# OpenDrift/opendrift

Measured on AMD Instinct MI355X. Metric: particle-steps/sec (RK4, 3D interp), higher is better.
Workload: dtype f64; 1 GPU; C3: OceanDrift 3D, synthetic ROMS-shaped z-level grid 1024x1024x12 (u,v,w,K), RK4 + vertical_mixing(60 s) + vertical_advection; particles_per_gpu=10000000, particles_total=10000000, stage_math=fast, spin_up_steps=200, block_every=0, inputs=resident in HBM, parallelism=particle-sharded x1, field block broadcast once per time level

## Files before the change

include/odrift.h:

```cpp
#ifndef ODRIFT_H
#define ODRIFT_H
#include <stdint.h>

#ifdef __cplusplus
extern "C" {
#endif

typedef struct odr_ctx odr_ctx;
typedef struct odr_particles odr_particles;

typedef enum {
  ODR_OK = 0,
  ODR_ERR_INVALID = -1,
  ODR_ERR_HIP = -2,
  ODR_ERR_CAPACITY = -3,
  ODR_ERR_STATE = -4
} odr_status;

enum {
  ODR_VAR_X_SEA_WATER_VELOCITY = 0,
  ODR_VAR_Y_SEA_WATER_VELOCITY = 1,
  ODR_VAR_X_WIND = 2,
  ODR_VAR_Y_WIND = 3,
  ODR_VAR_UPWARD_SEA_WATER_VELOCITY = 4,
// ... 252 lines not shown
                         const double *depth_noise, uint64_t step);
int odr_radio_terminal_velocity(odr_ctx *ctx, odr_particles *p, int diameter_slot, int density_slot);
int odr_radio_resuspend(odr_ctx *ctx, odr_particles *p, odr_radio *radio, int specie_slot, int diameter_slot, int rng_mode,
                        const double *diameter_noise, const double *depth_noise, uint64_t step);
int odr_particles_count_status(odr_ctx *ctx, odr_particles *p, int32_t status_code, int64_t *n);
int odr_particles_remap_status(odr_ctx *ctx, odr_particles *p, int32_t from_code, int32_t to_code);
int odr_deactivate(odr_ctx *ctx, odr_particles *p, const uint8_t *mask_host, int32_t status_code);
int odr_deactivate_outside(odr_ctx *ctx, odr_particles *p, double west, double east, double south, double north,
                           int32_t status_code);
int odr_compact(odr_ctx *ctx, odr_particles *p, int64_t *n_active);
int odr_scan_status(odr_ctx *ctx, odr_particles *p, int64_t *n_kept, uint64_t *status_flags);
int odr_scan_status_begin(odr_ctx *ctx, odr_particles *p);
int odr_scan_status_end(odr_ctx *ctx, odr_particles *p, int64_t *n_kept, uint64_t *status_flags);
int odr_ctx_guard_next_vmix(odr_ctx *ctx, int on);
int odr_compact_apply(odr_ctx *ctx, odr_particles *p, int64_t *n_active);
int odr_sort_particles(odr_ctx *ctx, odr_particles *p, int32_t source_id);
int odr_sort_particles_ex(odr_ctx *ctx, odr_particles *p, int32_t source_id, int keep_environment);
int odr_particles_tile_stats(odr_ctx *ctx, odr_particles *p, uint64_t *out4);
int odr_particles_step_layout_stats(odr_ctx *ctx, odr_particles *p, uint64_t *out2);
int odr_particles_step_onlevel_stats(odr_ctx *ctx, odr_particles *p, uint64_t *out1);
int odr_particles_vmix_layout_stats(odr_ctx *ctx, odr_particles *p, uint64_t *out3);
int odr_particles_vmix_kplane_stats(odr_ctx *ctx, odr_particles *p, uint64_t *out2);
int odr_particles_vmix_window_stats(odr_ctx *ctx, odr_particles *p, uint64_t *out3);
int odr_reduce_scalars(odr_ctx *ctx, odr_particles *p, double wind_drift_depth, double *out16);
int odr_ctx_set_step_reduce(odr_ctx *ctx, int on, double wind_drift_depth, int relative_wind);
int odr_reduce_local(odr_ctx *ctx, odr_particles *p, double wind_drift_depth, int relative_wind, double *out16);
int odr_reduce_install(odr_ctx *ctx, odr_particles *p, const double *in16);
int odr_reduce_unpin(odr_ctx *ctx);

int odr_ctx_set_position_class(odr_ctx *ctx, int f32);
int odr_source_set_coordinate_dtype(odr_ctx *ctx, int32_t source_id, int x_is_float32, int y_is_float32);

#define ODR_COMM_ID_BYTES 256
int odr_device_count(int32_t *n);
int odr_comm_unique_id(uint8_t *id );
int odr_comm_init(odr_ctx *ctx, const uint8_t *id, int32_t rank, int32_t nranks);
int odr_comm_info(int32_t *rank, int32_t *nranks, uint64_t *id_hash, int32_t *rccl_version, uint64_t *collectives);
int odr_comm_destroy(void);
int odr_allreduce_scalars(odr_ctx *ctx, double *values, int32_t n, int32_t op);
int odr_comm_allgather_begin(odr_ctx *ctx, const double *row, int32_t n, int32_t from_scan);
int odr_comm_allgather_end(odr_ctx *ctx, double *rows );
int odr_comm_broadcast_bytes(odr_ctx *ctx, void *buf, int64_t nbytes, int32_t root);
int odr_comm_barrier(odr_ctx *ctx);
int odr_block_broadcast(odr_ctx *ctx, int32_t source_id, int32_t slot, double t_epoch, int nvars, const int32_t *var_ids,
                        const void *const *data, const int32_t *var_nz, int ny, int nx, const double *xy8, int32_t root);

// ... 107 lines not shown
```

opendrift_amd/_abi.py:

```python
import ctypes as C
import os

HERE = os.path.dirname(os.path.abspath(__file__))
LIB_PATH = os.environ.get('ODR_LIB') or os.path.join(HERE, 'libodrift_hip.so')

NVAR = 26
VARIABLES = {
    'x_sea_water_velocity': 0, 'y_sea_water_velocity': 1, 'x_wind': 2, 'y_wind': 3,
    'upward_sea_water_velocity': 4, 'ocean_vertical_diffusivity': 5,
    'sea_surface_wave_stokes_drift_x_velocity': 6, 'sea_surface_wave_stokes_drift_y_velocity': 7,
    'land_binary_mask': 8, 'sea_floor_depth_below_sea_level': 9, 'sea_surface_height': 10,
    'horizontal_diffusivity': 11, 'sea_surface_wave_significant_height': 12,
    'sea_surface_wave_period_at_variance_spectral_density_maximum': 13,
    'ocean_mixed_layer_thickness': 14,
    'sea_water_temperature': 15, 'sea_water_salinity': 16,
    'sea_ice_area_fraction': 17, 'sea_ice_x_velocity': 18, 'sea_ice_y_velocity': 19,
    'sea_surface_swell_wave_to_direction': 20,
    'sea_surface_swell_wave_peak_period_from_variance_spectral_density': 21,
    'sea_surface_swell_wave_significant_height': 22, 'sea_surface_wind_wave_to_direction': 23,
    'sea_surface_wind_wave_mean_period': 24, 'sea_surface_wind_wave_significant_height': 25,
}
VARIABLE_NAMES = {v: k for k, v in VARIABLES.items()}
PROJ_LATLONG, PROJ_STERE_EQUIT_SPHERE, PROJ_STERE_POLAR = 0, 1, 2
PROJ_MERC, PROJ_LCC = 4, 5
# ... 158 lines not shown
    'odr_comm_unique_id': [_P(C.c_uint8)],
    'odr_comm_init': [_vp, _P(C.c_uint8), C.c_int32, C.c_int32],
    'odr_comm_info': [_P(C.c_int32), _P(C.c_int32), _P(C.c_uint64), _P(C.c_int32), _P(C.c_uint64)],
    'odr_comm_destroy': [],
    'odr_allreduce_scalars': [_vp, _dp, C.c_int32, C.c_int32],
    'odr_comm_allgather_begin': [_vp, _dp, C.c_int32, C.c_int32],
    'odr_comm_allgather_end': [_vp, _dp],
    'odr_comm_broadcast_bytes': [_vp, _vp, C.c_int64, C.c_int32],
    'odr_comm_barrier': [_vp],
    'odr_block_broadcast': [_vp, C.c_int32, C.c_int32, C.c_double, C.c_int, _ip, _P(_vp), _ip, C.c_int, C.c_int, _dp, C.c_int32],
    'odr_scan_status': [_vp, _vp, _i64p, _P(C.c_uint64)],
    'odr_scan_status_begin': [_vp, _vp],
    'odr_scan_status_end': [_vp, _vp, _i64p, _P(C.c_uint64)],
    'odr_ctx_guard_next_vmix': [_vp, C.c_int],
    'odr_compact_apply': [_vp, _vp, _i64p],
    'odr_sort_particles': [_vp, _vp, C.c_int32],
    'odr_sort_particles_ex': [_vp, _vp, C.c_int32, C.c_int],
    'odr_particles_tile_stats': [_vp, _vp, _P(C.c_uint64)],
    'odr_particles_step_layout_stats': [_vp, _vp, _P(C.c_uint64)],
    'odr_particles_step_onlevel_stats': [_vp, _vp, _P(C.c_uint64)],
    'odr_particles_vmix_layout_stats': [_vp, _vp, _P(C.c_uint64)],
    'odr_particles_vmix_kplane_stats': [_vp, _vp, _P(C.c_uint64)],
    'odr_particles_vmix_window_stats': [_vp, _vp, _P(C.c_uint64)],
    'odr_reduce_scalars': [_vp, _vp, C.c_double, _dp],
    'odr_ctx_set_step_reduce': [_vp, C.c_int, C.c_double, C.c_int],
    'odr_reduce_local': [_vp, _vp, C.c_double, C.c_int, _dp],
    'odr_reduce_install': [_vp, _vp, _dp],
    'odr_reduce_unpin': [_vp],
    'odr_timer_begin': [_vp],
    'odr_timer_end': [_vp, _fp],
    'odr_sgrid_create': [_vp, C.c_int32, C.c_int32, C.c_int32, _dp, _dp, C.c_double, _dp, _dp, C.c_int32, _P(_vp)],
    'odr_sgrid_destroy': [_vp, _vp],
    'odr_sgrid_download_zrho': [_vp, _vp, _dp],
    'odr_sgrid_zslice': [_vp, _vp, _vp, C.c_int, C.c_int, C.c_int32, _dp, C.c_int32, _P(_vp), _dp],
    'odr_history_create': [_vp, C.c_int64, C.c_int32, C.c_int32, _ip, _P(_vp)],
    'odr_history_destroy': [_vp, _vp],
    'odr_history_set_id_base': [_vp, _vp, C.c_int64],
    'odr_history_record': [_vp, _vp, _vp, C.c_int32, C.c_int, C.c_int],
    'odr_history_flush': [_vp, _vp, C.c_int32, C.c_int32],
    'odr_history_wait': [_vp, _vp],
    'odr_history_host_ptr': [_vp, _vp, C.c_int32, _P(_fp), _P(C.c_int32)],
    'odr_history_reset': [_vp, _vp],
    'odr_history_minmax': [_vp, _vp, C.c_int32, _dp, _dp],
    'odr_density_map': [_vp, C.c_int64, C.c_int32] + [_vp] * 5 + [C.c_int32, C.c_int32, _dp, C.c_int32, _dp, _dp, _dp, _dp],
    'odr_density_last_kernel_ms': [_vp, _fp],
    'odr_density_map_proj': [_vp, C.c_int64, C.c_int32] + [_vp] * 5 + [C.c_int32, _P(ProjDesc), C.c_int32, _dp, C.c_int32, _dp, C.c_int64, _dp, _dp, _dp],
# ... 81 lines not shown
```

opendrift_amd/build.py:

```python
import os
import subprocess
from concurrent.futures import ThreadPoolExecutor

HERE = os.path.dirname(os.path.abspath(__file__))
CSRC = os.path.join(HERE, 'csrc')
UNITS = sorted(f for f in os.listdir(CSRC) if f.endswith('.hip'))
HEADERS = sorted(os.path.join(CSRC, f) for f in os.listdir(CSRC) if f.endswith('.h')) + \
    [os.path.join(os.path.dirname(HERE), 'include', 'odrift.h')]
LIB = os.path.join(HERE, 'libodrift_hip.so')
OBJDIR = os.path.join(HERE, 'build')
HIPCC = os.environ.get('HIPCC', '/opt/rocm/bin/hipcc')
FLAGS = ['--offload-arch=gfx950', '-O3', '-std=c++17', '-ffp-contract=off', '-fPIC',
         '-I' + os.path.join(os.path.dirname(HERE), 'include')]


def _stale(target, deps):
    return not os.path.exists(target) or any(os.path.getmtime(target) < os.path.getmtime(d) for d in deps)


def build(force=False, verbose=False, extra_flags=(), lib=LIB, objdir=OBJDIR):
    os.makedirs(objdir, exist_ok=True)
    jobs = []
    for u in UNITS:
        src = os.path.join(CSRC, u)
        obj = os.path.join(objdir, u.replace('.hip', '.o'))
        if force or _stale(obj, [src] + HEADERS):
            jobs.append([HIPCC] + FLAGS + list(extra_flags) + ['-c', src, '-o', obj])
    if jobs:
        def run(cmd):
            if verbose:
                print(' '.join(cmd))
            subprocess.check_call(cmd)
        with ThreadPoolExecutor(len(jobs)) as ex:
            list(ex.map(run, jobs))
    objs = [os.path.join(objdir, u.replace('.hip', '.o')) for u in UNITS]
    if jobs or _stale(lib, objs):
        cmd = [HIPCC, '--offload-arch=gfx950', '-shared', '-fPIC', '-o', lib] + objs
        if verbose:
            print(' '.join(cmd))
        subprocess.check_call(cmd)
    return lib


if __name__ == '__main__':
    import sys
    print(build(force='--force' in sys.argv, verbose=True))


def build_variant(tag, units, extra_flags, outdir=None):
    build()
    outdir = outdir or os.path.join(os.path.dirname(HERE), 'tools')
    objdir = os.path.join(outdir, '_obj' + tag)
    os.makedirs(objdir, exist_ok=True)

    def run(u):
        obj = os.path.join(objdir, u.replace('.hip', '.o'))
        subprocess.check_call([HIPCC] + FLAGS + list(extra_flags) + ['-c', os.path.join(CSRC, u), '-o', obj])
        return obj
    with ThreadPoolExecutor(len(units)) as ex:
        mine = dict(zip(units, ex.map(run, units)))
    objs = [mine.get(u, os.path.join(OBJDIR, u.replace('.hip', '.o'))) for u in UNITS]
    lib = os.path.join(outdir, '_lib%s.so' % tag)
    subprocess.check_call([HIPCC, '--offload-arch=gfx950', '-shared', '-fPIC', '-o', lib] + objs)
    return lib
```

opendrift_amd/csrc/odr_host.h:

```cpp
#pragma once
#include <hip/hip_runtime.h>

#include <algorithm>
#include <cmath>
#include <cstdarg>
#include <cstdio>
#include <cstdlib>
#include <cstring>
#include <initializer_list>
#include <string>
#include <vector>

#include "../../include/odrift.h"
#include "odr_kernels.hip.h"

using namespace odr;

#include <chrono>
struct SlowSpan {
  const char *what;
  std::chrono::steady_clock::time_point t0;
  static double limit() { static const double v = getenv("ODR_SLOW_CALLS") ? atof(getenv("ODR_SLOW_CALLS")) : 0.0; return v; }
  explicit SlowSpan(const char *w) : what(w) { if (limit() > 0) t0 = std::chrono::steady_clock::now(); }
  ~SlowSpan() {
// ... 108 lines not shown
  double *dead64[3];
  int *deadi32[2];
  unsigned *bcount;
  unsigned *wcount;
  unsigned long long wcount_epoch;
  long long wcount_n;
  void *scratch;
  size_t scratch_bytes;
  unsigned long long epoch;
  unsigned long long status_epoch, scan_epoch;
  long long scan_kept;
  float env_cval[NVAR];
  long long env_cn[NVAR];
  bool env_cok[NVAR];
  bool external;
  unsigned *wg_tab, *wg_list;
  unsigned long long *wg_total, *wg_stats;
  long long wg_cap, wg_grid, wg_n, wg_list_cap;
  unsigned long long wg_launches;
  unsigned long long step_launches[3];
  unsigned long long vmix_launches[3];
  unsigned long long vmix_kplane[2];
  unsigned long long vmix_window[2];
  unsigned long long *vmix_redone;
  double *z_keep;
  long long z_keep_n;
  bool z_truncated;
  int wg_sid;
  bool wg_valid;
  unsigned wg_src_gen;
};

static inline unsigned nblk(long long n) { return (unsigned)((n + BLOCK - 1) / BLOCK); }

static inline PView view(const odr_particles *p) {
  PView v;
  v.n = p->n;
  v.lon = p->d64[0]; v.lat = p->d64[1]; v.z = p->d64[2]; v.plon = p->d64[3]; v.plat = p->d64[4];
  v.slon = p->d64[5]; v.slat = p->d64[6];
  v.id = p->i32[0]; v.status = p->i32[1]; v.moving = p->i32[2];
  v.wdf = p->f32[0]; v.cdf = p->f32[1]; v.tv = p->f32[2]; v.age = p->f32[3];
  for (int k = 0; k < NVAR; ++k) v.env[k] = p->env[k];
  for (int k = 0; k < 9; ++k) v.aux[k] = p->aux[k];
  v.ice = p->ice_kind; v.pad = 0;
  v.rank = p->rank_on && p->rank ? p->rank : nullptr;
  return v;
// ... 180 lines not shown
```

opendrift_amd/csrc/odr_kernels.hip.h:

```cpp
#pragma once
#include <hip/hip_runtime.h>
#include <rocrand/rocrand_kernel.h>
#include "odr_field.hip.h"

namespace odr {

#ifndef ODR_BLOCK
#define ODR_BLOCK 256
#endif
constexpr int BLOCK = ODR_BLOCK;
#ifndef ODR_POLAR_WAVES
#define ODR_POLAR_WAVES 3
#endif
#ifndef ODR_POLAR_STEP_WAVES
#define ODR_POLAR_STEP_WAVES 2
#endif
#define ODR_STEP_WAVES(PROJ) ((PROJ) == PROJ_LATLONG ? ODR_LATLONG_WAVES : ((PROJ) == PROJ_EXT ? 1 : ODR_POLAR_STEP_WAVES))
#ifndef ODR_LATLONG_WAVES
#define ODR_LATLONG_WAVES 1
#endif
#define ODR_WAVES(PROJ) ((PROJ) == PROJ_LATLONG ? ODR_LATLONG_WAVES : ((PROJ) == PROJ_EXT ? 1 : ODR_POLAR_WAVES))

__device__ __forceinline__ long long pid() {
  const unsigned nb = gridDim.x, b = blockIdx.x, per = nb >> 3, rem = nb & 7u, x = b & 7u, j = b >> 3;
  const unsigned lb = x * per + (x < rem ? x : rem) + j;
  return (long long)lb * BLOCK + threadIdx.x;
}

struct PView {
  long long n;
  double *lon, *lat, *z, *plon, *plat;
  double *slon, *slat;
  int *id, *status, *moving;
  float *wdf, *cdf, *tv, *age;
  float *aux[9];
  float *env[NVAR];
  int ice;
  int pad;
  const int *rank;
};

__device__ __forceinline__ int sf_species_flag(const PView &p, int sfl, long long i) {
  if ((sfl & 255) != 5) return 0;
  const int sp = (int)p.aux[(sfl >> 24) & 15][i];
  return (sp >= 0 && sp < 7 && (((sfl >> 8) >> sp) & 1)) ? 8 : 0;
}

__device__ __forceinline__ float ice_k(float A) {
  float k = __fdiv_rn(__fsub_rn(A, 0.3f), 0.5f);
  if (A < 0.3f) k = 0.f;
// ... 293 lines not shown
  return philox4x32<ODR_MIX_ROUNDS>(make_uint4(b, K.step_lo, K.id, K.tag), K.k0, K.k1);
}
__device__ __forceinline__ unsigned mix_word(const uint4 &q, unsigned k) {
  const unsigned lo = ((q.x & 255u) << 16) | ((q.y & 255u) << 8) | (q.z & 255u);
  return k == 0 ? q.x >> 8 : (k == 1 ? q.y >> 8 : (k == 2 ? q.z >> 8 : (k == 3 ? q.w >> 8 : lo)));
}
__device__ __forceinline__ unsigned mix_draw(const MixKey &K, uint4 &q, int it, bool primed = false) {
  const unsigned b = (unsigned)it / 5u, k = (unsigned)it - 5u * b;
  if (k == 0 && !(primed && it == 0)) q = mix_block(K, b);
  return mix_word(q, k);
}
__device__ __forceinline__ double mix_uniform(const MixKey &K, uint4 &q, int it, bool primed = false) {
  return ((double)mix_draw(K, q, it, primed) + 0.5) * 5.9604644775390625e-08;
}
__device__ __forceinline__ double mix_R_of(unsigned x) {
  return (double)((int)(2u * x + 1u) - (1 << 24)) * 5.9604644775390625e-08;
}
constexpr int AUX_KMEMBER = 8;
struct VMixDesc {
  int sid, nzp, geo_slot;
  unsigned kstride;
  const float *kb, *ka;
  double wgt;
  float Kfb, pad2;
  const unsigned long long *guard;
  unsigned long long *redone;
};

struct VMixRT {
  static constexpr bool STATIC = false;
  static constexpr bool WINDOW = false;
  __host__ __device__ static constexpr int proj_kind(int k) { return k; }
  __host__ __device__ static constexpr int lon_mode(int m) { return m; }
  __host__ __device__ static constexpr int mod360_x(int m) { return m; }
  __host__ __device__ static constexpr int nzp(int n, int ) { return n; }
  __host__ __device__ static constexpr bool uniform_z(bool u) { return u; }
  __host__ __device__ static constexpr int rng_mode(int m) { return m; }
  __host__ __device__ static constexpr int mix_at_surface(int m) { return m; }
  __host__ __device__ static constexpr int sf_action(int a) { return a; }
  __host__ __device__ static constexpr int vadv(int v) { return v; }
  __host__ __device__ static constexpr int ntimes(int n) { return n; }
  __host__ __device__ static constexpr unsigned kstride(unsigned b, int ) { return b; }
  __device__ static void proj_fwd(const DevProj &p, double lon, double lat, double &x, double &y) { proj_fwd_rt(p, lon, lat, x, y); }
};
struct VMixC3 {
  static constexpr bool STATIC = true;
  static constexpr bool WINDOW = false;
  __host__ __device__ static constexpr int proj_kind(int) { return PROJ_LATLONG; }
  __host__ __device__ static constexpr int lon_mode(int) { return 1; }
// ... 1298 lines not shown
}
template <int NQ, bool TL, class VM>
__device__ __forceinline__ bool vmix_col_particle(const DevSource &s, const PView &p, const VMixDesc &D, const VMixArgs &A,
                                                  int vadv, long long i, double *Kp, const double *gsh, int tid, const VMixState &S) {
  const int nzp = VM::nzp(D.nzp, 4 * NQ), sfl = A.sfl;
  const double dt = A.dt;
  const double slon = S.slon, slat = S.slat, z0 = S.z0;
  int moving = S.moving;
  const float dep0 = S.dep, ssh0 = S.ssh, tv0 = S.tv;
  const int id0 = S.id;
  MixRng R0;
  R0.key = mix_key(A.seed, A.step, id0); R0.q = make_uint4(0u, 0u, 0u, 0u); R0.primed = false;
  VMixWin win = {0, 0, false};
  if constexpr (VM::WINDOW) {
    double zm[4 * NQ - 1];
    vmix_level_bounds<4 * NQ>(s, nzp, zm);
    win.lv0 = vmix_start_level<4 * NQ>(zm, nzp, z0);
    const int qa = (win.lv0 > 2 ? win.lv0 - 2 : 0) >> 2;
    win.q0 = qa < NQ - 2 ? qa : NQ - 2;
  }
  vmix_col_fill<NQ, TL, VM>(s, D, slon, slat, Kp, tid, win.q0, [&]() { R0 = mix_rng_begin<VM>(A, id0); });
  int sf_flags = VM::sf_action(sfl & 255) == 5 ? sf_species_flag(p, sfl, i) : 0;
  const float Zmin = __fmul_rn(-1.f, __fadd_rn(dep0, ssh0));
  double z = vmix_col_walk<NQ, VM>(s, nzp, Kp, gsh, tid, A, i, p.n, id0, z0, moving, Zmin, tv0, sf_flags, &R0,
                                   VM::WINDOW ? &win : nullptr);
  if (VM::WINDOW && win.escaped) return true;
  if (sf_flags & 1) {
    if (p.status[i] == 0) p.status[i] = sfl >> 8;
    p.moving[i] = 0;
  }
  if (sf_flags & 4) p.moving[i] = 0;
  if (sf_flags & 2) { p.lon[i] = p.plon[i]; p.lat[i] = p.plat[i]; }
  vadv = VM::vadv(vadv);
  if (vadv >= 0 && (vadv ? z <= 0 : z < 0)) {
    const float w0 = p.env[VAR_W][i];
    double zz = __dadd_rn(z, __dmul_rn(__dmul_rn((double)moving, (double)w0), dt));
    z = zz < 0 ? zz : 0.0;
  }
  p.z[i] = z;
  return false;
}
template <int NQ, bool TL, class VM = VMixRT>
__global__ __launch_bounds__(BLOCK, ODR_VMIX_WAVES) void k_vmix_col(const DevWorld *__restrict__ W, PView p, VMixDesc D,
                                                    double dt, double dt_mix_cfg, int mix_at_surface,
                                                    int rng_mode, const double *__restrict__ huni,
                                                    unsigned long long seed, unsigned long long step,
                                                    int vadv, int sfl) {
  constexpr int NL = 4 * NQ;
  extern __shared__ __attribute__((aligned(16))) char smem[];
  const int tid = threadIdx.x;
  const DevSource &s = W->src[D.sid];
  const int nzp = VM::nzp(D.nzp, NL);
  double *Kp = (double *)smem;
  double *gsh = Kp + (size_t)NL * BLOCK;
  if (D.guard && *D.guard == 0ull) return;
  const long long i = pid();
  const bool valid = i < p.n;
  const VMixState S = vmix_load_state(p, valid ? i : 0);
  if (tid < nzp) {
    gsh[tid] = s.vg_a[tid]; gsh[NL + tid] = s.vg_b[tid]; gsh[2 * NL + tid] = s.vg_c[tid];
    gsh[3 * NL + tid] = s.zmid[tid];
  }
  __syncthreads();
  if (!valid) return;
  VMixArgs A;
  A.dt = dt; A.dt_mix_cfg = dt_mix_cfg; A.mix_at_surface = mix_at_surface; A.rng_mode = rng_mode; A.sfl = sfl; A.pad = 0;
  A.huni = huni; A.seed = seed; A.step = step;
  const bool escaped = vmix_col_particle<NQ, TL, VM>(s, p, D, A, vadv, i, Kp, gsh, tid, S);
  if constexpr (VM::WINDOW) {
    const unsigned long long esc = __ballot(escaped);
    if (esc != 0ull) {
      if (escaped) {
        const VMixState S2 = vmix_load_state(p, i);
        vmix_col_particle<NQ, TL, typename VM::Full>(s, p, D, A, vadv, i, Kp, gsh, tid, S2);
        if (D.redone && (tid & 63) == __ffsll((long long)esc) - 1) atomicAdd(D.redone, (unsigned long long)__popcll(esc));
      }
    }
  }
}

#ifndef ODR_VWIN_WAVES
#define ODR_VWIN_WAVES 5
#endif
template <bool TL>
__device__ __forceinline__ double vmix_layer(float b00, float b01, float b10, float b11, float a00, float a01, float a10, float a11,
                                             double w00, double w01, double w10, double w11, double wgt, bool cov, double Kfb) {
  double v = (double)bilw(b00, b01, b10, b11, w00, w01, w10, w11);
  if (TL) {
    const double w = (double)bilw(a00, a01, a10, a11, w00, w01, w10, w11);
    v = __dadd_rn(__dmul_rn(v, 1 - wgt), __dmul_rn(w, wgt));
  }
  return (cov && isfinite(v)) ? v : Kfb;
}
struct VMixGrad { double gd0, gi0, gd1, gi1, gd2, gi2, dt_mix; bool uniform_z; };
__device__ __forceinline__ void vmix_terms(const VMixGrad &G, const double *gsh, int nzp, int zl, double Kl, double Kz, double Kh,
                                           double &dk_dt, double &sg) {
  const double r = 1.0 / 3, ir = 1.0 / r;
  double gK;
// ... 1451 lines not shown
```

opendrift_amd/csrc/odr_mix.hip:

```cpp
#define ODR_TU_MIX 1
#include "odr_host.h"

template <class VM>
static bool vmix_layout_matches(const DevSource &s, const VMixDesc &D, int nq, double dt, double dt_mix, int mix_at_surface,
                                int rng_mode, int sfl, int vadv) {
  const bool uz = s.vg_uniform != 0;
  const int ntimes = abs((int)(dt / (dt_mix * (dt > 0 ? 1.0 : (dt < 0 ? -1.0 : 0.0)))));
  return VM::proj_kind(s.proj.kind) == s.proj.kind && VM::lon_mode(s.lon_mode) == s.lon_mode &&
         VM::mod360_x(s.mod360_x) == s.mod360_x && VM::nzp(D.nzp, 4 * nq) == D.nzp && VM::uniform_z(uz) == uz &&
         VM::rng_mode(rng_mode) == rng_mode && VM::mix_at_surface(mix_at_surface) == mix_at_surface &&
         VM::sf_action(sfl & 255) == (sfl & 255) && VM::vadv(vadv) == vadv && VM::ntimes(ntimes) == ntimes &&
         VM::kstride(D.kstride, nq) == D.kstride;
}

int odr_vmix(odr_ctx *c, odr_particles *p, double t, double dt, double dt_mix, int mix_at_surface, int rng_mode,
             const double *huni, uint64_t step) {
  const bool guarded = c->guard_next_vmix != 0;
  c->guard_next_vmix = 0;
  const bool oil = c->oil_owner == p;
  const bool f32prof = p->profiles_f32;
  const int cut = c->vmix_levels;
  VMixDesc D;
  bool kplanes = !getenv("ODR_NO_KPLANE");
  const bool fast = !oil && !f32prof && cut <= 0 && !getenv("ODR_NO_FAST_PATH") && build_vmix_desc(c, t, D, kplanes);
// ... 39 lines not shown
    ~F32ProfileClass() { if (on) { c->hw.f32pos &= ~2; c->dirty = true; } }
  } f32bit{c, false};
  if (f32prof) { c->hw.f32pos |= 2; c->dirty = true; f32bit.on = true; if ((rc = flush_world(c))) return rc; }
  if (cut > 0) {
    REQUIRE(cut >= 2 && cut <= 255, "odr_vmix_set_profile_levels: 2 .. 255 levels");
    if (cut < nzp) nzp = cut;
  }
  const int sfl_cut = c->seafloor | ((cut > 0 ? nzp : 0) << 16);
  if (fast) {
    if (guarded) { D.guard = c->counter + 4; c->guarded_vmix = p; c->guarded_vadv = vadv; }
    const int nq = (nzp + 3) / 4;
    const bool tl = D.ka != nullptr;
    const char *wenv = getenv("ODR_VMIX_WINDOW");
    const bool win = nzp >= 3 && nzp <= BLOCK && (wenv ? atoi(wenv) != 0 : nzp > 12);
    const bool spec = !win && (nq == 2 || nq == 3) &&
                      vmix_layout_matches<VMixC3Rec>(c->hw.src[D.sid], D, nq, dt, dt_mix, mix_at_surface, rng_mode, c->seafloor, vadv) &&
                      !getenv("ODR_NO_VMIX_SPEC");
    const bool specp = spec && vmix_layout_matches<VMixC3>(c->hw.src[D.sid], D, nq, dt, dt_mix, mix_at_surface, rng_mode, c->seafloor, vadv);
    const bool quadwin = spec && nq == 3 && !getenv("ODR_NO_VMIX_WINDOW");
    p->vmix_launches[win ? 2 : spec ? 1 : 0]++;
    p->vmix_kplane[kplanes ? 0 : 1]++;
    if (spec && nq == 3) p->vmix_window[quadwin ? 0 : 1]++;
    D.redone = quadwin ? p->vmix_redone : nullptr;
#define VMIX_COL(NQ, VM)                                                                                          \
  do {                                                                                                            \
    size_t l2 = sizeof(double) * ((size_t)(4 * NQ) * BLOCK + 4 * (size_t)(4 * NQ));                               \
    if (tl) hipLaunchKernelGGL((k_vmix_col<NQ, true, VM>), g, b, l2, c->stream, c->dw, v, D, dt, dt_mix,          \
                               mix_at_surface, rng_mode, du, c->seed, st, vadv, c->seafloor);                                  \
    else hipLaunchKernelGGL((k_vmix_col<NQ, false, VM>), g, b, l2, c->stream, c->dw, v, D, dt, dt_mix,            \
                            mix_at_surface, rng_mode, du, c->seed, st, vadv, c->seafloor);                                     \
  } while (0)
    if (win) {
      const size_t lw = (sizeof(double) + sizeof(unsigned)) * 4 * BLOCK + sizeof(double) * 4 * (size_t)nzp;
      if (tl) hipLaunchKernelGGL((k_vmix_win<true>), g, b, lw, c->stream, c->dw, v, D, dt, dt_mix, mix_at_surface, rng_mode, du,
                                 c->seed, st, vadv, c->seafloor);
      else hipLaunchKernelGGL((k_vmix_win<false>), g, b, lw, c->stream, c->dw, v, D, dt, dt_mix, mix_at_surface, rng_mode, du,
                              c->seed, st, vadv, c->seafloor);
    }
    else if (specp && nq == 2) VMIX_COL(2, VMixC3);
    else if (specp && quadwin) VMIX_COL(3, VMixC3W);
    else if (specp) VMIX_COL(3, VMixC3);
    else if (spec && nq == 2) VMIX_COL(2, VMixC3Rec);
    else if (spec && quadwin) VMIX_COL(3, VMixC3RecW);
    else if (spec) VMIX_COL(3, VMixC3Rec);
    else if (nq <= 1) VMIX_COL(1, VMixRT);
    else if (nq == 2) VMIX_COL(2, VMixRT);
    else if (nq == 3) VMIX_COL(3, VMixRT);
    else if (nq == 4) VMIX_COL(4, VMixRT);
    else if (nq <= 6) VMIX_COL(6, VMixRT);
// ... 5 lines not shown
    if (nzp <= 16) hipLaunchKernelGGL((k_vmix<16, true>), g, b, lds, c->stream, c->dw, v, t, dt, dt_mix, mix_at_surface, rng_mode, du, c->seed, st, vadv, sfl_cut, c->oil);
    else if (nzp <= 32) hipLaunchKernelGGL((k_vmix<32, true>), g, b, lds, c->stream, c->dw, v, t, dt, dt_mix, mix_at_surface, rng_mode, du, c->seed, st, vadv, sfl_cut, c->oil);
    else hipLaunchKernelGGL((k_vmix<1, true>), g, b, lds, c->stream, c->dw, v, t, dt, dt_mix, mix_at_surface, rng_mode, du, c->seed, st, vadv, sfl_cut, c->oil);
  } else if (nzp <= 16) hipLaunchKernelGGL(k_vmix<16>, g, b, lds, c->stream, c->dw, v, t, dt, dt_mix, mix_at_surface, rng_mode, du, c->seed, st, vadv, sfl_cut);
  else if (nzp <= 32) hipLaunchKernelGGL(k_vmix<32>, g, b, lds, c->stream, c->dw, v, t, dt, dt_mix, mix_at_surface, rng_mode, du, c->seed, st, vadv, sfl_cut);
  else hipLaunchKernelGGL(k_vmix<1>, g, b, lds, c->stream, c->dw, v, t, dt, dt_mix, mix_at_surface, rng_mode, du, c->seed, st, vadv, sfl_cut);
  if (!fast) p->vmix_launches[2]++;
  HIPCHK(hipGetLastError());
  return 0;
}

int odr_particles_vmix_layout_stats(odr_ctx *c, odr_particles *p, uint64_t *out3) {
  REQUIRE(c && p && out3, "NULL argument");
  for (int k = 0; k < 3; ++k) out3[k] = p->vmix_launches[k];
  return 0;
}

int odr_particles_vmix_kplane_stats(odr_ctx *c, odr_particles *p, uint64_t *out2) {
  REQUIRE(c && p && out2, "NULL argument");
  out2[0] = p->vmix_kplane[0]; out2[1] = p->vmix_kplane[1];
  return 0;
}

int odr_particles_vmix_window_stats(odr_ctx *c, odr_particles *p, uint64_t *out3) {
  REQUIRE(c && p && out3, "NULL argument");
  unsigned long long redone = 0;
  D2H(&redone, p->vmix_redone, sizeof redone);
  HIPCHK(hipStreamSynchronize(c->stream));
  out3[0] = p->vmix_window[0]; out3[1] = p->vmix_window[1]; out3[2] = redone;
  return 0;
}

int odr_vmix_set_profile_levels(odr_ctx *c, int32_t n) {
  REQUIRE(n == 0 || (n >= 2 && n <= 255), "bad level count %d", n);
  c->vmix_levels = n;
  return 0;
}

int odr_vmix_wind_profile(odr_ctx *c, odr_particles *p, int model, double background_diffusivity, double dt,
                          double dt_mix, int mix_at_surface, int rng_mode, const double *huni, uint64_t step) {
  c->guard_next_vmix = 0;
  p->status_epoch++;
  p->epoch++;
  REQUIRE(model == ODR_DIFFUSIVITY_LARGE1994 || model == ODR_DIFFUSIVITY_SUNDBY1983, "Unknown diffusivity model: %d", model);
  REQUIRE(dt_mix > 0 && dt != 0, "bad time steps");
  if (!p->env[VAR_DEPTH]) return fail(ODR_ERR_STATE, "sea_floor_depth_below_sea_level has not been sampled");
// ... 168 lines not shown
```

opendrift_amd/csrc/odrift.hip:

```cpp
#define ODR_TU_MISC 1
#include "odr_host.h"
#include "odr_mesh.h"

static thread_local std::string g_err;
int odr_i_fail(int code, const char *fmt, ...) {
  char buf[512];
  va_list ap;
  va_start(ap, fmt);
  vsnprintf(buf, sizeof buf, fmt, ap);
  va_end(ap);
  g_err = buf;
  return code;
}

const char *odr_last_error(void) { return g_err.c_str(); }
#define ODR_STR2(x) #x
#define ODR_STR(x) ODR_STR2(x)
const char *odr_version(void) { return "odrift-hip 0.2 (gfx950; mixing stream Philox4x32-" ODR_STR(ODR_MIX_ROUNDS) ")"; }

int odr_ctx_create(int device, uint64_t seed, odr_ctx **out) {
  REQUIRE(out, "out is NULL");
  HIPCHK(hipSetDevice(device));
  odr_ctx *c = new odr_ctx();
  c->device = device;
// ... 79 lines not shown
  return 0;
}
int odr_timer_end(odr_ctx *c, float *ms) {
  HIPCHK(hipEventRecord(c->ev1, c->stream));
  HIPCHK(hipEventSynchronize(c->ev1));
  HIPCHK(hipEventElapsedTime(ms, c->ev0, c->ev1));
  return 0;
}

int odr_particles_create(odr_ctx *c, int64_t capacity, odr_particles **out) {
  REQUIRE(capacity > 0 && out, "capacity must be positive");
  HIPCHK(hipSetDevice(c->device));
  odr_particles *p = new odr_particles();
  memset(p, 0, sizeof(*p));
  p->cap = capacity;
  p->dead_cap = capacity;
  p->scan_kept = -1;
  for (int k = 0; k < 7; ++k) HIPCHK(hipMalloc((void **)&p->d64[k], sizeof(double) * (size_t)capacity));
  for (int k = 0; k < 3; ++k) HIPCHK(hipMalloc((void **)&p->i32[k], sizeof(int) * (size_t)capacity));
  for (int k = 0; k < 4; ++k) HIPCHK(hipMalloc((void **)&p->f32[k], sizeof(float) * (size_t)capacity));
  HIPCHK(hipMalloc((void **)&p->bcount, sizeof(unsigned) * (size_t)(nblk(capacity) + 1)));
  HIPCHK(hipMalloc((void **)&p->wcount, sizeof(unsigned) * (size_t)(nblk(capacity) + 1) * (BLOCK / 64)));
  p->wcount_epoch = ~0ull;
  HIPCHK(hipMalloc((void **)&p->vmix_redone, sizeof(unsigned long long)));
  HIPCHK(hipMemset(p->vmix_redone, 0, sizeof(unsigned long long)));
  *out = p;
  return 0;
}

int odr_particles_destroy(odr_ctx *c, odr_particles *p) {
  if (c->red_owner == p) c->red_owner = nullptr;
  if (c->noise_owner == p) c->noise_owner = nullptr;
  if (c->guarded_vmix == p) c->guarded_vmix = nullptr;
  if (!p) return 0;
  (void)hipStreamSynchronize(c->stream);
  auto fr = [](void *q) { if (q) (void)hipFree(q); };
  for (int k = 0; k < 7; ++k) { fr(p->d64[k]); fr(p->alt64[k]); }
  for (int k = 0; k < 3; ++k) { fr(p->i32[k]); fr(p->alti32[k]); fr(p->dead64[k]); }
  for (int k = 0; k < 4; ++k) { fr(p->f32[k]); fr(p->altf32[k]); }
  for (int k = 0; k < 2; ++k) fr(p->deadi32[k]);
  for (int k = 0; k < NVAR; ++k) { fr(p->env[k]); fr(p->altenv[k]); }
  for (int k = 0; k < 9; ++k) { fr(p->aux[k]); fr(p->altaux[k]); fr(p->aux_snap[k]); }
  fr(p->bcount);
  fr(p->wcount);
  fr(p->vmix_redone);
  fr(p->scratch);
  fr(p->rank); fr(p->rank_words); fr(p->rank_before); fr(p->rank_bsum);
  fr(p->wg_tab); fr(p->wg_total); fr(p->wg_list); fr(p->z_keep);
// ... 2430 lines not shown
```

opendrift_amd/device.py:

```python
import ctypes as C
import os

import numpy as np

from . import _abi
from ._abi import VARIABLES, check

_dp, _fp, _ip = C.POINTER(C.c_double), C.POINTER(C.c_float), C.POINTER(C.c_int32)


def _vid(v, aliases=None):
    if isinstance(v, (int, np.integer)):
        return v
    if v in VARIABLES:
        return VARIABLES[v]
    if aliases and v in aliases:
        return aliases[v]
    raise KeyError(v)


def _d(a, n=None):
    if a is None:
        return None, None
    a = np.ascontiguousarray(np.broadcast_to(np.asarray(a, dtype=np.float64), (n,)) if n is not None
# ... 1177 lines not shown
        import ctypes as C
        out = (C.c_uint64 * 1)()
        check(self.lib.odr_particles_step_onlevel_stats(self.ctx.h, self.h, out))
        return int(out[0])

    def vmix_layout_stats(self):
        import ctypes as C
        out = (C.c_uint64 * 3)()
        check(self.lib.odr_particles_vmix_layout_stats(self.ctx.h, self.h, out))
        return dict(runtime=int(out[0]), static=int(out[1]), other=int(out[2]))

    def vmix_kplane_stats(self):
        import ctypes as C
        out = (C.c_uint64 * 2)()
        check(self.lib.odr_particles_vmix_kplane_stats(self.ctx.h, self.h, out))
        return dict(planes=int(out[0]), records=int(out[1]))

    def vmix_window_stats(self):
        import ctypes as C
        out = (C.c_uint64 * 3)()
        check(self.lib.odr_particles_vmix_window_stats(self.ctx.h, self.h, out))
        return dict(windowed=int(out[0]), full=int(out[1]), redone=int(out[2]))

    def reduce_global(self, combine, wind_drift_depth=0.1, relative_wind=False):
        raw = np.empty(16)
        check(self.lib.odr_reduce_local(self.ctx.h, self.h, float(wind_drift_depth), int(relative_wind), raw.ctypes.data_as(_dp)))
        g = np.ascontiguousarray(combine(raw), dtype=np.float64)
        check(self.lib.odr_reduce_install(self.ctx.h, self.h, g.ctypes.data_as(_dp)))
        return g

    def reduce_local(self, wind_drift_depth=0.1, relative_wind=False):
        raw = np.empty(16)
        check(self.lib.odr_reduce_local(self.ctx.h, self.h, float(wind_drift_depth), int(relative_wind), raw.ctypes.data_as(_dp)))
        return raw

    def reduce_install(self, combined16):
        g = np.ascontiguousarray(combined16, dtype=np.float64)
        check(self.lib.odr_reduce_install(self.ctx.h, self.h, g.ctypes.data_as(_dp)))

    @staticmethod
    def reduction_dict(raw):
        keys = ['n_active', 'lon_min', 'lon_max', 'lat_min', 'lat_max', 'z_min', 'z_max', 'D_max',
                'stokes_sum_max', 'wind_speed_max', 'wdf_surface_max', 'n_surface', 'hs_max', 'tp_max']
        d = dict(zip(keys, raw))
        for k in ('lon_min', 'lat_min', 'z_min'):
            d[k] = -d[k]
# ... 344 lines not shown
```

Measured before the change: 11.92 billion particle-steps/s.

## Tile vertical-mixing kernel and compact out surface-pinned particles before the column walk

The vertical-mixing column kernel now assigns each workgroup a tile of several blocks' worth of particles, first scans them to find particles sitting at z==0 with mixing at the surface disabled (which would stay at the surface), and builds a compacted LDS index list of the remaining particles that then walk the column in dense waves. This aims to avoid wasting lanes on trivially unchanged particles and improves wave utilisation, at the cost of extra LDS, a prefix-count step and an indirect index. It also adds a skip counter, an env opt-out, readfirstlane pinning of uniform scalars, and disables machine LICM for the mix unit to control register pressure.

```diff
diff --git a/include/odrift.h b/include/odrift.h
--- a/include/odrift.h
+++ b/include/odrift.h
@@ -298,6 +298,7 @@
 int odr_particles_vmix_layout_stats(odr_ctx *ctx, odr_particles *p, uint64_t *out3);
 int odr_particles_vmix_kplane_stats(odr_ctx *ctx, odr_particles *p, uint64_t *out2);
 int odr_particles_vmix_window_stats(odr_ctx *ctx, odr_particles *p, uint64_t *out3);
+int odr_particles_vmix_skip_stats(odr_ctx *ctx, odr_particles *p, uint64_t *out2);
 int odr_reduce_scalars(odr_ctx *ctx, odr_particles *p, double wind_drift_depth, double *out16);
 int odr_ctx_set_step_reduce(odr_ctx *ctx, int on, double wind_drift_depth, int relative_wind);
 int odr_reduce_local(odr_ctx *ctx, odr_particles *p, double wind_drift_depth, int relative_wind, double *out16);
diff --git a/opendrift_amd/_abi.py b/opendrift_amd/_abi.py
--- a/opendrift_amd/_abi.py
+++ b/opendrift_amd/_abi.py
@@ -204,6 +204,7 @@
     'odr_particles_vmix_layout_stats': [_vp, _vp, _P(C.c_uint64)],
     'odr_particles_vmix_kplane_stats': [_vp, _vp, _P(C.c_uint64)],
     'odr_particles_vmix_window_stats': [_vp, _vp, _P(C.c_uint64)],
+    'odr_particles_vmix_skip_stats': [_vp, _vp, _P(C.c_uint64)],
     'odr_reduce_scalars': [_vp, _vp, C.c_double, _dp],
     'odr_ctx_set_step_reduce': [_vp, C.c_int, C.c_double, C.c_int],
     'odr_reduce_local': [_vp, _vp, C.c_double, C.c_int, _dp],
diff --git a/opendrift_amd/build.py b/opendrift_amd/build.py
--- a/opendrift_amd/build.py
+++ b/opendrift_amd/build.py
@@ -12,6 +12,7 @@
 HIPCC = os.environ.get('HIPCC', '/opt/rocm/bin/hipcc')
 FLAGS = ['--offload-arch=gfx950', '-O3', '-std=c++17', '-ffp-contract=off', '-fPIC',
          '-I' + os.path.join(os.path.dirname(HERE), 'include')]
+UNIT_FLAGS = {'odr_mix.hip': ['-mllvm', '-disable-machine-licm']}
 
 
 def _stale(target, deps):
@@ -25,7 +26,7 @@
         src = os.path.join(CSRC, u)
         obj = os.path.join(objdir, u.replace('.hip', '.o'))
         if force or _stale(obj, [src] + HEADERS):
-            jobs.append([HIPCC] + FLAGS + list(extra_flags) + ['-c', src, '-o', obj])
+            jobs.append([HIPCC] + FLAGS + UNIT_FLAGS.get(u, []) + list(extra_flags) + ['-c', src, '-o', obj])
     if jobs:
         def run(cmd):
             if verbose:
@@ -55,7 +56,7 @@
 
     def run(u):
         obj = os.path.join(objdir, u.replace('.hip', '.o'))
-        subprocess.check_call([HIPCC] + FLAGS + list(extra_flags) + ['-c', os.path.join(CSRC, u), '-o', obj])
+        subprocess.check_call([HIPCC] + FLAGS + UNIT_FLAGS.get(u, []) + list(extra_flags) + ['-c', os.path.join(CSRC, u), '-o', obj])
         return obj
     with ThreadPoolExecutor(len(units)) as ex:
         mine = dict(zip(units, ex.map(run, units)))
diff --git a/opendrift_amd/csrc/odr_host.h b/opendrift_amd/csrc/odr_host.h
--- a/opendrift_amd/csrc/odr_host.h
+++ b/opendrift_amd/csrc/odr_host.h
@@ -154,6 +154,7 @@
   unsigned long long vmix_launches[3];
   unsigned long long vmix_kplane[2];
   unsigned long long vmix_window[2];
+  unsigned long long vmix_tiled;
   unsigned long long *vmix_redone;
   double *z_keep;
   long long z_keep_n;
diff --git a/opendrift_amd/csrc/odr_kernels.hip.h b/opendrift_amd/csrc/odr_kernels.hip.h
--- a/opendrift_amd/csrc/odr_kernels.hip.h
+++ b/opendrift_amd/csrc/odr_kernels.hip.h
@@ -21,11 +21,11 @@
 #endif
 #define ODR_WAVES(PROJ) ((PROJ) == PROJ_LATLONG ? ODR_LATLONG_WAVES : ((PROJ) == PROJ_EXT ? 1 : ODR_POLAR_WAVES))
 
-__device__ __forceinline__ long long pid() {
+__device__ __forceinline__ unsigned pid_wg() {
   const unsigned nb = gridDim.x, b = blockIdx.x, per = nb >> 3, rem = nb & 7u, x = b & 7u, j = b >> 3;
-  const unsigned lb = x * per + (x < rem ? x : rem) + j;
-  return (long long)lb * BLOCK + threadIdx.x;
-}
+  return x * per + (x < rem ? x : rem) + j;
+}
+__device__ __forceinline__ long long pid() { return (long long)pid_wg() * BLOCK + threadIdx.x; }
 
 struct PView {
   long long n;
@@ -365,9 +365,11 @@
   unsigned kstride;
   const float *kb, *ka;
   double wgt;
-  float Kfb, pad2;
+  float Kfb;
+  int noskip;
   const unsigned long long *guard;
   unsigned long long *redone;
+  unsigned long long *skipped;
 };
 
 struct VMixRT {
@@ -1712,7 +1714,8 @@
   vmix_col_fill<NQ, TL, VM>(s, D, slon, slat, Kp, tid, win.q0, [&]() { R0 = mix_rng_begin<VM>(A, id0); });
   int sf_flags = VM::sf_action(sfl & 255) == 5 ? sf_species_flag(p, sfl, i) : 0;
   const float Zmin = __fmul_rn(-1.f, __fadd_rn(dep0, ssh0));
-  double z = vmix_col_walk<NQ, VM>(s, nzp, Kp, gsh, tid, A, i, p.n, id0, z0, moving, Zmin, tv0, sf_flags, &R0,
+  const float tv1 = VM::STATIC ? tv0 : p.tv[i];
+  double z = vmix_col_walk<NQ, VM>(s, nzp, Kp, gsh, tid, A, i, p.n, id0, z0, moving, Zmin, tv1, sf_flags, &R0,
                                    VM::WINDOW ? &win : nullptr);
   if (VM::WINDOW && win.escaped) return true;
   if (sf_flags & 1) {
@@ -1730,40 +1733,127 @@
   p.z[i] = z;
   return false;
 }
+constexpr int VMIX_TILE_ROUNDS = 4;
+constexpr int VMIX_TILE = VMIX_TILE_ROUNDS * BLOCK;
+static_assert(VMIX_TILE <= 65536, "tile-relative offsets are 16 bits");
+__host__ __device__ constexpr size_t vmix_col_lds_bytes(int nq) {
+  return sizeof(double) * ((size_t)(4 * nq) * BLOCK + 4 * (size_t)(4 * nq)) + sizeof(unsigned short) * VMIX_TILE +
+         sizeof(unsigned) * VMIX_TILE_ROUNDS * (BLOCK / 64);
+}
+__device__ __forceinline__ float vmix_per_pass(float v) {
+  asm volatile("" : "+v"(v));
+  return __int_as_float(__builtin_amdgcn_readfirstlane(__float_as_int(v)));
+}
+__device__ __forceinline__ double vmix_per_pass(double v) {
+  asm volatile("" : "+v"(v));
+  const long long b = __double_as_longlong(v);
+  const unsigned lo = (unsigned)__builtin_amdgcn_readfirstlane((int)b), hi = (unsigned)__builtin_amdgcn_readfirstlane((int)(b >> 32));
+  return __longlong_as_double((long long)(((unsigned long long)hi << 32) | lo));
+}
 template <int NQ, bool TL, class VM = VMixRT>
 __global__ __launch_bounds__(BLOCK, ODR_VMIX_WAVES) void k_vmix_col(const DevWorld *__restrict__ W, PView p, VMixDesc D,
                                                     double dt, double dt_mix_cfg, int mix_at_surface,
                                                     int rng_mode, const double *__restrict__ huni,
                                                     unsigned long long seed, unsigned long long step,
                                                     int vadv, int sfl) {
-  constexpr int NL = 4 * NQ;
+  constexpr int NL = 4 * NQ, NW = BLOCK / 64;
   extern __shared__ __attribute__((aligned(16))) char smem[];
-  const int tid = threadIdx.x;
-  const DevSource &s = W->src[D.sid];
+  const int tid = threadIdx.x, lane = tid & 63, wave = tid >> 6;
   const int nzp = VM::nzp(D.nzp, NL);
   double *Kp = (double *)smem;
   double *gsh = Kp + (size_t)NL * BLOCK;
+  unsigned short *list = (unsigned short *)(gsh + 4 * NL);
+  unsigned *cnt = (unsigned *)(list + VMIX_TILE);
   if (D.guard && *D.guard == 0ull) return;
-  const long long i = pid();
-  const bool valid = i < p.n;
-  const VMixState S = vmix_load_state(p, valid ? i : 0);
+  const long long base = (long long)pid_wg() * VMIX_TILE;
+  const bool may_skip = VM::mix_at_surface(mix_at_surface) == 0 && VM::vadv(vadv) != 1 && !D.noskip;
+  unsigned long long keep[VMIX_TILE_ROUNDS];
+  if (may_skip) {
+    double z[VMIX_TILE_ROUNDS];
+    float dep[VMIX_TILE_ROUNDS], ssh[VMIX_TILE_ROUNDS];
+#pragma unroll
+    for (int r = 0; r < VMIX_TILE_ROUNDS; ++r) {
+      const long long e = base + r * BLOCK + tid, ec = e < p.n ? e : 0;
+      z[r] = p.z[ec]; dep[r] = p.env[VAR_DEPTH][ec]; ssh[r] = p.env[VAR_SSH][ec];
+    }
+    const double sgn = dt > 0 ? 1.0 : (dt < 0 ? -1.0 : 0.0);
+    const bool walks = VM::ntimes(abs((int)(dt / (dt_mix_cfg * sgn)))) > 0;
+#pragma unroll
+    for (int r = 0; r < VMIX_TILE_ROUNDS; ++r) {
+      const long long e = base + r * BLOCK + tid;
+      const float Zmin = __fmul_rn(-1.f, __fadd_rn(dep[r], ssh[r]));
+      const bool skip = e < p.n && z[r] == 0 && !(Zmin > 0.f);
+      if (skip && walks && __double_as_longlong(z[r]) != 0ll) p.z[e] = 0.0;
+      keep[r] = __ballot(e < p.n && !skip);
+    }
+  } else {
+#pragma unroll
+    for (int r = 0; r < VMIX_TILE_ROUNDS; ++r) keep[r] = __ballot(base + r * BLOCK + tid < p.n);
+  }
+  if (lane == 0) {
+#pragma unroll
+    for (int r = 0; r < VMIX_TILE_ROUNDS; ++r) cnt[r * NW + wave] = (unsigned)__popcll(keep[r]);
+  }
   if (tid < nzp) {
+    const DevSource &s = W->src[D.sid];
     gsh[tid] = s.vg_a[tid]; gsh[NL + tid] = s.vg_b[tid]; gsh[2 * NL + tid] = s.vg_c[tid];
     gsh[3 * NL + tid] = s.zmid[tid];
   }
   __syncthreads();
-  if (!valid) return;
-  VMixArgs A;
-  A.dt = dt; A.dt_mix_cfg = dt_mix_cfg; A.mix_at_surface = mix_at_surface; A.rng_mode = rng_mode; A.sfl = sfl; A.pad = 0;
-  A.huni = huni; A.seed = seed; A.step = step;
-  const bool escaped = vmix_col_particle<NQ, TL, VM>(s, p, D, A, vadv, i, Kp, gsh, tid, S);
-  if constexpr (VM::WINDOW) {
-    const unsigned long long esc = __ballot(escaped);
-    if (esc != 0ull) {
-      if (escaped) {
-        const VMixState S2 = vmix_load_state(p, i);
-        vmix_col_particle<NQ, TL, typename VM::Full>(s, p, D, A, vadv, i, Kp, gsh, tid, S2);
-        if (D.redone && (tid & 63) == __ffsll((long long)esc) - 1) atomicAdd(D.redone, (unsigned long long)__popcll(esc));
+  unsigned total = 0, off[VMIX_TILE_ROUNDS];
+#pragma unroll
+  for (int r = 0; r < VMIX_TILE_ROUNDS; ++r) {
+#pragma unroll
+    for (int w = 0; w < NW; ++w) {
+      if (w == wave) off[r] = total;
+      total += cnt[r * NW + w];
+    }
+  }
+  if (tid == 0 && D.skipped) {
+    const long long left = p.n - base;
+    const unsigned in_tile = left < (long long)VMIX_TILE ? (unsigned)left : (unsigned)VMIX_TILE;
+    if (in_tile > total) atomicAdd(D.skipped, (unsigned long long)(in_tile - total));
+  }
+  total = __builtin_amdgcn_readfirstlane(total);
+  if (total == 0) return;
+  const unsigned long long below = (1ull << lane) - 1ull;
+#pragma unroll
+  for (int r = 0; r < VMIX_TILE_ROUNDS; ++r)
+    if ((keep[r] >> lane) & 1ull) list[off[r] + (unsigned)__popcll(keep[r] & below)] = (unsigned short)(r * BLOCK + tid);
+  __syncthreads();
+  const DevSource &s = W->src[D.sid];
+  const unsigned wave0 = (unsigned)__builtin_amdgcn_readfirstlane(tid - lane);
+#pragma unroll 1
+  for (unsigned e0 = 0; e0 + wave0 < total; e0 += BLOCK) {
+    VMixDesc Dp = D;
+    Dp.wgt = vmix_per_pass(D.wgt); Dp.Kfb = vmix_per_pass(D.Kfb);
+    VMixArgs A;
+    A.dt = vmix_per_pass(dt); A.dt_mix_cfg = vmix_per_pass(dt_mix_cfg);
+    A.mix_at_surface = mix_at_surface; A.rng_mode = rng_mode; A.sfl = sfl; A.pad = 0;
+    A.huni = huni; A.seed = seed; A.step = step;
+    int t;
+    asm volatile("v_mbcnt_lo_u32_b32 %0, -1, 0\n\tv_mbcnt_hi_u32_b32 %0, -1, %0" : "=&v"(t));
+    t += (int)wave0;
+    const unsigned e = e0 + (unsigned)t;
+    long long i = 0;
+    bool escaped = false;
+    if (e < total) {
+      i = base + list[e];
+      long long i1 = i;
+      asm volatile("" : "+v"(i1));
+      const VMixState S = vmix_load_state(p, i1);
+      escaped = vmix_col_particle<NQ, TL, VM>(s, p, Dp, A, vadv, i, Kp, gsh, t, S);
+    }
+    if constexpr (VM::WINDOW) {
+      const unsigned long long esc = __ballot(escaped);
+      if (esc != 0ull) {
+        if (escaped) {
+          long long i2 = i;
+          asm volatile("" : "+v"(i2));
+          const VMixState S2 = vmix_load_state(p, i2);
+          vmix_col_particle<NQ, TL, typename VM::Full>(s, p, Dp, A, vadv, i, Kp, gsh, t, S2);
+          if (D.redone && (t & 63) == __ffsll((long long)esc) - 1) atomicAdd(D.redone, (unsigned long long)__popcll(esc));
+        }
       }
     }
   }
diff --git a/opendrift_amd/csrc/odr_mix.hip b/opendrift_amd/csrc/odr_mix.hip
--- a/opendrift_amd/csrc/odr_mix.hip
+++ b/opendrift_amd/csrc/odr_mix.hip
@@ -1,5 +1,7 @@
 #define ODR_TU_MIX 1
 #include "odr_host.h"
+
+static_assert(vmix_col_lds_bytes(3) <= 163840 / ODR_VMIX_WAVES, "k_vmix_col<3>: column, tables and offset list exceed a sixth of the LDS");
 
 template <class VM>
 static bool vmix_layout_matches(const DevSource &s, const VMixDesc &D, int nq, double dt, double dt_mix, int mix_at_surface,
@@ -85,9 +87,12 @@
     p->vmix_kplane[kplanes ? 0 : 1]++;
     if (spec && nq == 3) p->vmix_window[quadwin ? 0 : 1]++;
     D.redone = quadwin ? p->vmix_redone : nullptr;
+    D.skipped = p->vmix_redone + 1;
+    D.noskip = getenv("ODR_NO_VMIX_SKIP") ? 1 : 0;
+    if (!win) { g = dim3((unsigned)((p->n + VMIX_TILE - 1) / VMIX_TILE)); p->vmix_tiled++; }
 #define VMIX_COL(NQ, VM)                                                                                          \
   do {                                                                                                            \
-    size_t l2 = sizeof(double) * ((size_t)(4 * NQ) * BLOCK + 4 * (size_t)(4 * NQ));                               \
+    const size_t l2 = vmix_col_lds_bytes(NQ);                                                                     \
     if (tl) hipLaunchKernelGGL((k_vmix_col<NQ, true, VM>), g, b, l2, c->stream, c->dw, v, D, dt, dt_mix,          \
                                mix_at_surface, rng_mode, du, c->seed, st, vadv, c->seafloor);                                  \
     else hipLaunchKernelGGL((k_vmix_col<NQ, false, VM>), g, b, l2, c->stream, c->dw, v, D, dt, dt_mix,            \
@@ -139,6 +144,15 @@
   return 0;
 }
 
+int odr_particles_vmix_skip_stats(odr_ctx *c, odr_particles *p, uint64_t *out2) {
+  REQUIRE(c && p && out2, "NULL argument");
+  unsigned long long skipped = 0;
+  D2H(&skipped, p->vmix_redone + 1, sizeof skipped);
+  HIPCHK(hipStreamSynchronize(c->stream));
+  out2[0] = p->vmix_tiled; out2[1] = skipped;
+  return 0;
+}
+
 int odr_particles_vmix_window_stats(odr_ctx *c, odr_particles *p, uint64_t *out3) {
   REQUIRE(c && p && out3, "NULL argument");
   unsigned long long redone = 0;
diff --git a/opendrift_amd/csrc/odrift.hip b/opendrift_amd/csrc/odrift.hip
--- a/opendrift_amd/csrc/odrift.hip
+++ b/opendrift_amd/csrc/odrift.hip
@@ -125,8 +125,8 @@
   HIPCHK(hipMalloc((void **)&p->bcount, sizeof(unsigned) * (size_t)(nblk(capacity) + 1)));
   HIPCHK(hipMalloc((void **)&p->wcount, sizeof(unsigned) * (size_t)(nblk(capacity) + 1) * (BLOCK / 64)));
   p->wcount_epoch = ~0ull;
-  HIPCHK(hipMalloc((void **)&p->vmix_redone, sizeof(unsigned long long)));
-  HIPCHK(hipMemset(p->vmix_redone, 0, sizeof(unsigned long long)));
+  HIPCHK(hipMalloc((void **)&p->vmix_redone, 2 * sizeof(unsigned long long)));
+  HIPCHK(hipMemset(p->vmix_redone, 0, 2 * sizeof(unsigned long long)));
   *out = p;
   return 0;
 }
diff --git a/opendrift_amd/device.py b/opendrift_amd/device.py
--- a/opendrift_amd/device.py
+++ b/opendrift_amd/device.py
@@ -1223,6 +1223,12 @@
         check(self.lib.odr_particles_vmix_window_stats(self.ctx.h, self.h, out))
         return dict(windowed=int(out[0]), full=int(out[1]), redone=int(out[2]))
 
+    def vmix_skip_stats(self):
+        import ctypes as C
+        out = (C.c_uint64 * 2)()
+        check(self.lib.odr_particles_vmix_skip_stats(self.ctx.h, self.h, out))
+        return dict(launches=int(out[0]), skipped=int(out[1]))
+
     def reduce_global(self, combine, wind_drift_depth=0.1, relative_wind=False):
         raw = np.empty(16)
         check(self.lib.odr_reduce_local(self.ctx.h, self.h, float(wind_drift_depth), int(relative_wind), raw.ctypes.data_as(_dp)))
```

New measurement: 12.27 billion particle-steps/s (median of 6 runs). 1.03x the previous value.
